# kotaro-kinoshita/yomitoku

Measured on AMD Instinct MI355X. Metric: pages/sec (DocumentAnalyzer @1600x1200, lite model set), higher is better.
Workload: dtype f32 held as two scaled fp16 planes per operand on the MFMA pipe: 3 x v_mfma_f32_32x32x16_f16 per product tile (products to 2^-21, below the fp32 accumulation's own rounding), fp32 accumulate, fp32 activations in HBM; attention, LayerNorm, the fused greedy step and every grid-starved launch exact fp3

## Files before the change

yomitoku_amd/csrc/ymk_api.cpp:

```cpp
#include "../../include/ymk.h"
#include "ymk_common.h"
#include "ymk_decstep.h"
#include "ymk_det.h"
#include "ymk_entry.h"
#include "ymk_seq.h"

struct ymk_model {
  ymk::Model* impl = nullptr;
  int device = 0;
};

#include <dlfcn.h>
namespace {
struct Roctx {
  int (*push)(const char*) = nullptr;
  int (*pop)() = nullptr;
  Roctx() {
    const char* on = std::getenv("YMK_ROCTX");
    if (on == nullptr || on[0] == '\0' || on[0] == '0') return;
    for (const char* name : {"librocprofiler-sdk-roctx.so", "libroctx64.so"}) {
      if (void* h = dlopen(name, RTLD_NOW | RTLD_GLOBAL)) {
        push = reinterpret_cast<int (*)(const char*)>(dlsym(h, "roctxRangePushA"));
        pop = reinterpret_cast<int (*)()>(dlsym(h, "roctxRangePop"));
        if (push && pop) return;
// ... 26 lines not shown
    return 1;                                       \
  }                                                 \
  catch (...) {                                     \
    ymk::set_error("unknown C++ exception");        \
    return 2;                                       \
  }

extern "C" {

int ymk_version(void) { return 100; }

const char* ymk_last_error(void) { return ymk::last_error().c_str(); }

int ymk_device_count(void) {
  int n = 0;
  if (hipGetDeviceCount(&n) != hipSuccess) return -1;
  return n;
}

ymk_model* ymk_model_create(const char* kind, int device) {
  try {
    YMK_CHECK(kind != nullptr, "kind is null");
    YMK_HIP(hipSetDevice(device));
    std::string k(kind);
    ymk::Model* impl = nullptr;
    if (k == "dbnet") impl = ymk::create_dbnet();
    else if (k == "parseq") impl = ymk::create_parseq();
    else if (k == "rtdetr") impl = ymk::create_rtdetr();
    else throw ymk::Error("unknown model kind: " + k);
    auto* m = new ymk_model();
    m->impl = impl;
    m->device = device;
    return m;
  } catch (const std::exception& e) {
    ymk::set_error(e.what());
    return nullptr;
  }
}

void ymk_model_destroy(ymk_model* m) {
  if (!m) return;
  (void)hipSetDevice(m->device);
  delete m->impl;
  delete m;
}

int ymk_model_set_param(ymk_model* m, const char* key, double value) {
  YMK_API_BEGIN
  YMK_CHECK(m && key, "null argument");
  const std::string k(key);
  if (k == "workspace_reuse") {
    YMK_CHECK(value == 0.0 || value == 1.0 || value == -1.0, "workspace_reuse must be 0 or 1 (-1: follow the process-wide default)");
    YMK_CHECK(!ymk::in_forward(), "workspace_reuse cannot change inside a forward");
  }
  m->impl->params[key] = value;
  if (m->impl->finalized && (k == "conv_split" || k == "conv_split_encoder")) {
    YMK_HIP(hipSetDevice(m->device));
    m->impl->prebuild_split();
  }
  YMK_API_END
}

int ymk_model_set_tensor(ymk_model* m, const char* name, const float* host_data, int ndim, const int64_t* dims) {
  YMK_API_BEGIN
  YMK_CHECK(m && name && host_data && (ndim == 0 || dims), "null argument");
  YMK_CHECK(!m->impl->finalized, "model already finalized");
  m->impl->ws.put(name, host_data, ndim, dims);
  YMK_API_END
}

int ymk_model_finalize(ymk_model* m) {
  YMK_API_BEGIN
  RoctxRange roctx_range("ymk_model_finalize");
  YMK_CHECK(m, "null model");
  YMK_HIP(hipSetDevice(m->device));
  m->impl->finalize();
  m->impl->prebuild_split();
  if (!ymk::debug_hazard_no_finalize_sync()) YMK_HIP(hipDeviceSynchronize());
  YMK_API_END
}

int ymk_model_reserve(ymk_model* m, int n, int h, int w, void* stream) {
  YMK_API_BEGIN
  RoctxRange roctx_range("ymk_model_reserve");
  YMK_CHECK(m && m->impl, "null argument");
  YMK_HIP(hipSetDevice(m->device));
  m->impl->reserve(n, h, w, (hipStream_t)stream);
  YMK_API_END
}

int64_t ymk_model_weight_bytes(const ymk_model* m) { return m ? (int64_t)m->impl->pool.bytes() : -1; }
int64_t ymk_model_workspace_bytes(const ymk_model* m) { return m ? (int64_t)m->impl->arena.capacity() : -1; }

int ymk_dbnet_forward(ymk_model* m, const float* x_dev, int n, int h, int w, float* prob_dev, void* stream) {
  YMK_API_BEGIN
  RoctxRange roctx_range("ymk_dbnet_forward");
  YMK_CHECK(m && x_dev && prob_dev, "null argument");
  YMK_HIP(hipSetDevice(m->device));
  ymk::dbnet_forward(m->impl, x_dev, n, h, w, prob_dev, (hipStream_t)stream);
  YMK_API_END
}

int ymk_parseq_dims(ymk_model* m, int* num_steps, int* num_classes) {
  YMK_API_BEGIN
  YMK_CHECK(m && num_steps && num_classes, "null argument");
  ymk::parseq_dims(m->impl, num_steps, num_classes);
  YMK_API_END
}

int ymk_parseq_forward(ymk_model* m, const float* x_dev, int b, int w, float* logits_dev, int* out_len, int* ar_steps,
                       void* stream) {
  YMK_API_BEGIN
  RoctxRange roctx_range("ymk_parseq_forward");
  YMK_CHECK(m && x_dev && logits_dev && out_len && ar_steps, "null argument");
  YMK_HIP(hipSetDevice(m->device));
  ymk::parseq_forward(m->impl, x_dev, b, w, logits_dev, out_len, ar_steps, (hipStream_t)stream);
  YMK_API_END
}

int ymk_parseq_forward_groups(ymk_model* m, const float* const* x_dev, const int* b, const int* w, int n_groups,
                              float* logits_dev, int* out_len, int* ar_steps, void* stream) {
  YMK_API_BEGIN
  RoctxRange roctx_range("ymk_parseq_forward_groups");
  YMK_CHECK(m && x_dev && b && w && logits_dev && out_len && ar_steps, "null argument");
  YMK_HIP(hipSetDevice(m->device));
  ymk::parseq_forward_groups(m->impl, x_dev, b, w, n_groups, logits_dev, out_len, ar_steps, (hipStream_t)stream);
  YMK_API_END
}

int ymk_parseq_token_stats(const float* logits_dev, int rows, int num_classes, int* ids_dev, float* probs_dev,
                           void* stream) {
  YMK_API_BEGIN
  RoctxRange roctx_range("ymk_parseq_token_stats");
  YMK_CHECK(logits_dev && ids_dev && probs_dev, "null argument");
  ymk::row_maxprob((hipStream_t)stream, logits_dev, rows, num_classes, ids_dev, probs_dev);
  YMK_API_END
}

int ymk_rtdetr_forward(ymk_model* m, const float* x_dev, int b, int h, int w, float* logits_dev, float* boxes_dev,
                       void* stream) {
  YMK_API_BEGIN
  RoctxRange roctx_range("ymk_rtdetr_forward");
  YMK_CHECK(m && x_dev && logits_dev && boxes_dev, "null argument");
  YMK_HIP(hipSetDevice(m->device));
  ymk::rtdetr_forward(m->impl, x_dev, b, h, w, logits_dev, boxes_dev, (hipStream_t)stream);
  YMK_API_END
}

int ymk_debug_option(const char* key, int value) {
  YMK_API_BEGIN
  YMK_CHECK(key != nullptr, "null key");
  const std::string k(key);
  YMK_CHECK(ymk::conv_debug_option(k, value) || ymk::parseq_debug_option(k, value) || ymk::decstep_debug_option(k, value) ||
                ymk::conv_split_debug_option(k, value) || ymk::runtime_debug_option(k, value),
            "unknown debug option: " + k);
  YMK_API_END
}

int ymk_stat(const char* key, int64_t* value) {
  YMK_API_BEGIN
  YMK_CHECK(key != nullptr && value != nullptr, "null argument");
  long long v = 0;
  YMK_CHECK(ymk::conv_split_stat(std::string(key), &v) || ymk::runtime_stat(std::string(key), &v) || ymk::parseq_stat(std::string(key), &v), std::string("unknown counter: ") + key);
  *value = v;
  YMK_API_END
}

int ymk_amax_check_counters(int64_t* out4) {
  YMK_API_BEGIN
  YMK_CHECK(out4 != nullptr, "null argument");
  long long v[4];
  ymk::amax_check_counters(v);
  for (int i = 0; i < 4; ++i) out4[i] = v[i];
  YMK_API_END
}

int ymk_prof_begin(void) {
  YMK_API_BEGIN
  ymk::prof_begin();
  YMK_API_END
}

int ymk_prof_end(double* conv_ms, double* conv_flop, int64_t* conv_launches) {
  YMK_API_BEGIN
  YMK_CHECK(conv_ms && conv_flop && conv_launches, "null argument");
  ymk::prof_end(conv_ms, conv_flop, conv_launches);
  YMK_API_END
}

int ymk_prof_bytes(double* conv_bytes) {
  YMK_API_BEGIN
  YMK_CHECK(conv_bytes, "null argument");
  *conv_bytes = ymk::prof_bytes();
  YMK_API_END
}

int ymk_prof_launch_table(double* ms, double* flop, double* bytes, double* mfma_products, int64_t capacity, int64_t* count) {
  YMK_API_BEGIN
  YMK_CHECK(count != nullptr && capacity >= 0 && (capacity == 0 || (ms && flop && bytes && mfma_products)), "null argument");
  *count = ymk::prof_launch_table(ms, flop, bytes, mfma_products, capacity);
  YMK_API_END
}

int ymk_op_plan_workspace(int64_t n, const int64_t* sizes, const int64_t* release_pos, int64_t* offsets_out, int64_t* peak_out,
                          int64_t* live_bound_out) {
  YMK_API_BEGIN
  YMK_CHECK(n >= 0 && (n == 0 || (sizes && offsets_out)), "plan_workspace: bad argument");
  std::vector<size_t> sz((size_t)n), off((size_t)n);
  for (int64_t k = 0; k < n; ++k) {
    YMK_CHECK(sizes[k] >= 0, "plan_workspace: negative size");
    sz[(size_t)k] = (size_t)sizes[k];
  }
  size_t peak = 0, live = 0;
  ymk::plan_workspace((size_t)n, sz.data(), release_pos, off.data(), &peak, &live);
  for (int64_t k = 0; k < n; ++k) offsets_out[k] = (int64_t)off[(size_t)k];
  if (peak_out) *peak_out = (int64_t)peak;
  if (live_bound_out) *live_bound_out = (int64_t)live;
  YMK_API_END
}

int ymk_op_conv2d(const float* x_dev, int n, int h, int w, int c, const float* w_host_oihw, int cout, int cin, int kh,
                  int kw, const float* scale_host, const float* bias_host, const float* res_dev, int stride, int pad,
                  int dil, int act, int tap4, float* y_dev, void* stream) {
  YMK_API_BEGIN
  using namespace ymk;
  DevicePool pool;
  ConvW cw;
  cw.cout = cout;
  cw.cin = tap4 ? 4 : cin;
  cw.kh = kh;
  cw.kw = kw;
  cw.mode = tap4 ? 1 : 0;
  std::vector<float> panel;
  pack_conv_weight(w_host_oihw, cout, cin, kh, kw, tap4 != 0, panel, cw.kpad, cw.ctiles);
  cw.w = pool.upload(panel);
  if (scale_host) cw.scale = pool.upload(scale_host, cout);
  if (bias_host) cw.bias = pool.upload(bias_host, cout);
  Tensor in{const_cast<float*>(x_dev), n, h, w, c, c};
  const int oh = conv_out_dim(h, kh, stride, pad, dil), ow = conv_out_dim(w, kw, stride, pad, dil);
  Tensor out{y_dev, n, oh, ow, cout, cout};
  Tensor res{const_cast<float*>(res_dev), n, oh, ow, cout, cout};
  ConvArgs a;
  a.stride = stride;
  a.pad = pad;
  a.dil = dil;
  a.act = act;
  a.res = res_dev ? &res : nullptr;
  SplitCtxOwner split_ctx;
  ConvSplitScope scope(-1, split_ctx.get(), 0);
  conv2d((hipStream_t)stream, in, cw, a, out);
  YMK_HIP(hipStreamSynchronize((hipStream_t)stream));
  YMK_API_END
}

static ymk::ConvW op_conv_weight(ymk::DevicePool& pool, const float* w_host_oihw, int cout, int cin, int kh, int kw, bool tap4,
                                 const float* scale_host, const float* bias_host) {
  using namespace ymk;
  ConvW cw;
  cw.cout = cout;
  cw.cin = tap4 ? 4 : cin;
  cw.kh = kh;
  cw.kw = kw;
  cw.mode = tap4 ? 1 : 0;
  std::vector<float> panel;
  pack_conv_weight(w_host_oihw, cout, cin, kh, kw, tap4, panel, cw.kpad, cw.ctiles);
  cw.w = pool.upload(panel);
  std::vector<float> scale, bias;
  if (scale_host) scale.assign(scale_host, scale_host + cout);
  if (bias_host) bias.assign(bias_host, bias_host + cout);
  if (scale_host) cw.scale = pool.upload(scale);
  if (bias_host) cw.bias = pool.upload(bias);
  plane_bound(cw, w_host_oihw, (size_t)cin * kh * kw, scale, bias);
  return cw;
}

int ymk_op_conv2d_view(const float* x_dev, int n, int h, int w, int c, int in_ld, const float* w_host_oihw, int cout, int kh, int kw,
                       int tap4, const float* scale_host, const float* bias_host, const float* res_dev, int res_ld, int res_post,
                       int stride_h, int stride_w, int pad, int dil, int act, const int* row_group_dev, const int* group_open_dev,
                       const unsigned* amax_in_dev, unsigned* amax_out_dev, float* y_dev, int out_ld, void* stream) {
  YMK_API_BEGIN
  using namespace ymk;
  YMK_CHECK(x_dev && w_host_oihw && y_dev, "null argument");
  YMK_CHECK(n > 0 && h > 0 && w > 0 && c > 0 && in_ld > 0 && cout > 0 && kh > 0 && kw > 0 && res_ld >= 0 && out_ld > 0 &&
                stride_h > 0 && stride_w > 0 && pad >= 0 && dil > 0,
            "conv2d_view: sizes, strides and leading dimensions are positive (res_ld may be 0)");
  hipStream_t s = (hipStream_t)stream;
  DevicePool pool;
  const ConvW cw = op_conv_weight(pool, w_host_oihw, cout, c, kh, kw, tap4 != 0, scale_host, bias_host);
  SplitCtxOwner split_ctx;
  ConvSplitScope scope(-1, split_ctx.get(), 0);
  if (row_group_dev || group_open_dev) {
    YMK_CHECK(kh == 1 && kw == 1 && stride_h == 1 && stride_w == 1 && pad == 0 && !res_post && !tap4,
              "conv2d_view: a row predicate comes with a plain linear layer");
    gemm(s, x_dev, n * h * w, c, in_ld, cw, act, res_dev, res_ld, y_dev, out_ld, row_group_dev, group_open_dev, EPI_STORE, amax_in_dev,
         amax_out_dev);
  } else {
    Tensor in{const_cast<float*>(x_dev), n, h, w, c, in_ld};
    const int oh = conv_out_dim(h, kh, stride_h, pad, dil), ow = conv_out_dim(w, kw, stride_w, pad, dil);
    Tensor out{y_dev, n, oh, ow, cout, out_ld};
    Tensor res{const_cast<float*>(res_dev), n, oh, ow, cout, res_ld};
    ConvArgs a;
    a.stride = stride_h;
    a.stride_w = stride_w;
    a.pad = pad;
    a.dil = dil;
    a.act = act;
    a.res = res_dev ? &res : nullptr;
    a.res_post = res_post != 0;
    a.amax_in = amax_in_dev;
    a.amax_out = amax_out_dev;
    conv2d(s, in, cw, a, out);
  }
  YMK_HIP(hipStreamSynchronize(s));
  YMK_API_END
}

// ... 515 lines not shown
```

yomitoku_amd/csrc/ymk_seq.h:

```cpp
#pragma once
#include "ymk_common.h"

namespace ymk {

void layernorm(hipStream_t s, const float* x, int ldx, int in_rows_mod, const float* g, const float* b, float eps,
               float* y, int ldy, int M, int D);
void add_pos_embed(hipStream_t s, float* x, const float* pos, int B, int gh, int gw, int full_gw, int D);

struct SeqTab {
  const int *qoff = nullptr, *qlen = nullptr, *koff = nullptr, *klen = nullptr;
};

void flash_attention(hipStream_t s, const float* q, const float* k, const float* v, float* o, int B, int H, int Lq, int Lk,
                     int hd, int ldq, int ldk, int ldv, int ldo, long bsq, long bsk, long bsv, long bso, float scale,
                     const SeqTab* tab = nullptr, const unsigned* amax_q = nullptr, const unsigned* amax_k = nullptr,
                     const unsigned* amax_v = nullptr);
void small_attention(hipStream_t s, const float* q, const float* k, const float* v, float* o, int B, int H, int Lq, int Lk,
                     int hd, int ldq, int ldk, int ldv, int ldo, long bsq, long bsk, long bsv, long bso, float scale,
                     const unsigned char* mask_qk, int ld_mask, const unsigned char* kpm, int ld_kpm,
                     const SeqTab* tab = nullptr);
void nar_cross_attention(hipStream_t s, const float* q, const float* k, const float* v, float* o, int B, int H, int Lq, int Lk,
                         int hd, int ldq, int ldk, int ldv, int ldo, long bsk, long bsv, long bso, float scale,
                         const SeqTab* tab = nullptr);
void init_decode(hipStream_t s, int* tok, int ld_tok, int* state, int bos_id, int pad_id, int B);

void ctx_embed_ln(hipStream_t s, const int* tok, int ld_tok, int pos0, int npos, const float* emb, const float* posq,
                  const float* g, const float* be, float eps, float* out, int out_rows, int D, int B);
void greedy_step(hipStream_t s, const float* logits, long ld_b, int C, int step, int num_steps, int* tok, int* raw,
                 int ld_tok, int* state, int eos_id, int rep_on, int period_max, int min_run_p1, int min_repeats,
                 int* not_done, const int* prev_not_done, int* arrived, int* host_flag, int B, const int* gid = nullptr,
                 int* gopen = nullptr, int ng = 1, int partials = 0);
void publish_open(hipStream_t s, const int* not_done, const int* prev_not_done, int* host_flag);
void refine_prep(hipStream_t s, const int* raw, int ld_tok, int S, int bos_id, int eos_id, int* tok2, unsigned char* kpm,
                 int B, const int* gid = nullptr, const int* gsteps = nullptr);
void row_argmax(hipStream_t s, const float* logits, int rows, int C, int* out);
void rep_cut(hipStream_t s, float* logits, long ld_b, int C, int S, const int* state, int eos_id, int B);
void row_maxprob(hipStream_t s, const float* logits, int rows, int C, int* ids, float* probs);
void tile_rows(hipStream_t s, const float* src, int rows, int D, float* dst, int B);
void fill_i32(hipStream_t s, int* p, int v, size_t n);

}
```

yomitoku_amd/csrc/ymk_seq.hip:

```cpp
#include "ymk_common.h"
#include "ymk_f16_planes.h"
#include "ymk_seq.h"

namespace ymk {


__device__ __forceinline__ float wave_sum(float v) {
#pragma unroll
  for (int o = 32; o > 0; o >>= 1) v += __shfl_xor(v, o, 64);
  return v;
}
__device__ __forceinline__ float wave_max(float v) {
#pragma unroll
  for (int o = 32; o > 0; o >>= 1) v = fmaxf(v, __shfl_xor(v, o, 64));
  return v;
}

__global__ void k_layernorm(const float* __restrict__ x, int ldx, int in_rows_mod, const float* __restrict__ g,
                            const float* __restrict__ b, float eps, float* __restrict__ y, int ldy, int M, int D) {
  const int row = blockIdx.x * (blockDim.x >> 6) + (threadIdx.x >> 6);
  const int lane = threadIdx.x & 63;
  if (row >= M) return;
  const float* xr = x + (size_t)(in_rows_mod > 0 ? row % in_rows_mod : row) * ldx;
  float4 v[4];
  const int nv = D >> 2;
  float s = 0.f;
#pragma unroll
  for (int i = 0; i < 4; ++i) {
    const int c = lane + 64 * i;
    if (c < nv) {
      v[i] = *reinterpret_cast<const float4*>(xr + c * 4);
      s += (v[i].x + v[i].y) + (v[i].z + v[i].w);
    }
  }
  const float mean = wave_sum(s) / (float)D;
  float q = 0.f;
#pragma unroll
  for (int i = 0; i < 4; ++i) {
    const int c = lane + 64 * i;
    if (c < nv) {
      const float a = v[i].x - mean, bb = v[i].y - mean, cc = v[i].z - mean, d = v[i].w - mean;
      q += (a * a + bb * bb) + (cc * cc + d * d);
    }
  }
  const float rstd = 1.f / sqrtf(wave_sum(q) / (float)D + eps);
#pragma unroll
  for (int i = 0; i < 4; ++i) {
    const int c = lane + 64 * i;
    if (c < nv) {
      const float4 gg = *reinterpret_cast<const float4*>(g + c * 4);
      const float4 be = *reinterpret_cast<const float4*>(b + c * 4);
      float4 o;
      o.x = (v[i].x - mean) * rstd * gg.x + be.x;
      o.y = (v[i].y - mean) * rstd * gg.y + be.y;
      o.z = (v[i].z - mean) * rstd * gg.z + be.z;
      o.w = (v[i].w - mean) * rstd * gg.w + be.w;
      *reinterpret_cast<float4*>(y + (size_t)row * ldy + c * 4) = o;
    }
  }
}
void layernorm(hipStream_t s, const float* x, int ldx, int in_rows_mod, const float* g, const float* b, float eps,
               float* y, int ldy, int M, int D) {
  YMK_CHECK(D % 4 == 0 && D <= 1024, "layernorm: D must be a multiple of 4, <= 1024");
  if (M == 0) return;
  hipLaunchKernelGGL(k_layernorm, dim3((M + 3) / 4), dim3(256), 0, s, x, ldx, in_rows_mod, g, b, eps, y, ldy, M, D);
  YMK_HIP(hipGetLastError());
}

__global__ void k_add_pos(float* __restrict__ x, const float* __restrict__ pos, int gh, int gw, int full_gw, int D4,
                          size_t total) {
  for (size_t i = (size_t)blockIdx.x * blockDim.x + threadIdx.x; i < total; i += (size_t)gridDim.x * blockDim.x) {
    const int c4 = (int)(i % D4);
    const size_t tok = i / D4;
    const int cc = (int)(tok % gw);
    const int rr = (int)((tok / gw) % gh);
    float4 v = reinterpret_cast<float4*>(x)[i];
    const float4 p = reinterpret_cast<const float4*>(pos)[(size_t)(rr * full_gw + cc) * D4 + c4];
    v.x += p.x; v.y += p.y; v.z += p.z; v.w += p.w;
    reinterpret_cast<float4*>(x)[i] = v;
  }
}
void add_pos_embed(hipStream_t s, float* x, const float* pos, int B, int gh, int gw, int full_gw, int D) {
  const size_t total = (size_t)B * gh * gw * (D / 4);
  size_t g = (total + 255) / 256;
  if (g > 4096) g = 4096;
  hipLaunchKernelGGL(k_add_pos, dim3((int)g), dim3(256), 0, s, x, pos, gh, gw, full_gw, D / 4, total);
  YMK_HIP(hipGetLastError());
}

struct AttnP {
  const float *q, *k, *v;
  float* o;
  int ldq, ldk, ldv, ldo;
  long bsq, bsk, bsv, bso;
  int Lq, Lk, H;
  float scale;
  const int *qoff, *qlen, *koff, *klen;
  const unsigned *amax_q, *amax_k, *amax_v;
};

template <int HD, int HDR = HD>
__global__ __launch_bounds__(256, 1) void k_flash_attn(AttnP p) {
  constexpr int KT = 64;
  constexpr int LDH = HD + 4;
  constexpr int NKC = HDR / 8;
  constexpr int NDC = HD / 32;
  constexpr int LPT = (KT * HDR / 4) / 256;
  static_assert(HD % 32 == 0 && HDR % 8 == 0 && HDR <= HD && (KT * HDR / 4) % 256 == 0, "head dim");
  __shared__ __attribute__((aligned(16))) float lds[2 * 2 * KT * LDH];

  const int t = threadIdx.x, wv = t >> 6, lane = t & 63, li = lane & 31, lh = lane >> 5;
  const int b = blockIdx.z, h = blockIdx.y;
  const int q0 = blockIdx.x * 128 + wv * 32;
  const float* qb = p.q + (size_t)b * p.bsq + h * HDR;
  const float* kb = p.k + (size_t)b * p.bsk + h * HDR;
  const float* vb = p.v + (size_t)b * p.bsv + h * HDR;
  float* ob = p.o + (size_t)b * p.bso + h * HDR;
  int Lq = p.Lq, Lk = p.Lk;
  if (p.koff) {
    const size_t r = (size_t)p.koff[b];
    kb = p.k + r * p.ldk + h * HDR;
    vb = p.v + r * p.ldv + h * HDR;
    Lk = p.klen[b];
  }
  if (p.qoff) {
    const size_t r = (size_t)p.qoff[b];
    qb = p.q + r * p.ldq + h * HDR;
    ob = p.o + r * p.ldo + h * HDR;
    Lq = p.qlen[b];
  }
  if ((int)blockIdx.x * 128 >= Lq) return;

  f32x4 qf[NKC];
  {
    const int qi = min(q0 + li, Lq - 1);
    const float* qr = qb + (size_t)qi * p.ldq;
#pragma unroll
    for (int kc = 0; kc < NKC; ++kc) {
      qf[kc] = *reinterpret_cast<const f32x4*>(qr + kc * 8 + lh * 4);
      qf[kc] *= p.scale;
    }
  }

  f32x16 oacc[NDC];
#pragma unroll
  for (int dc = 0; dc < NDC; ++dc)
#pragma unroll
    for (int r = 0; r < 16; ++r) oacc[dc][r] = 0.f;
  float m_run = -INFINITY, l_run = 0.f;

  f32x4 rk[LPT], rv[LPT];
  auto load_kv = [&](int k0) {
// ... 172 lines not shown
    for (int i = 0; i < LPT; ++i) {
      const int idx = t + 256 * i;
      const int row = idx / (HDR / 4), c4 = idx - row * (HDR / 4);
      *reinterpret_cast<f32x4*>(Ks + row * LDH + c4 * 4) = rk[i];
      *reinterpret_cast<f32x4*>(Vs + row * LDH + c4 * 4) = rv[i];
    }
  };

  const int ntiles = (Lk + KT - 1) / KT;
  load_kv(0);
  store_kv(0);
  __syncthreads();
  for (int tt = 0; tt < ntiles; ++tt) {
    const int buf = tt & 1;
    if (tt + 1 < ntiles) load_kv((tt + 1) * KT);
    const float* Ks = lds + buf * (2 * KT * LDH);
    const float* Vs = Ks + KT * LDH;
#pragma unroll
    for (int sub = 0; sub < (q0 < Lq ? KT / 32 : 0); ++sub) {
      const int kbase = tt * KT + sub * 32;
      if (kbase >= Lk) break;
      f32x16 sacc;
#pragma unroll
      for (int r = 0; r < 16; ++r) sacc[r] = 0.f;
      const float* kr = Ks + (sub * 32 + li) * LDH + lh * 8;
#pragma unroll
      for (int ks = 0; ks < NKS; ++ks) {
        const f32x4 a = *reinterpret_cast<const f32x4*>(kr + ks * 16);
        const f32x4 c = *reinterpret_cast<const f32x4*>(kr + ks * 16 + 4);
        const float x[8] = {a.x, a.y, a.z, a.w, c.x, c.y, c.z, c.w};
        f16x8 kh, kl;
        f16_split8(x, s_k, kh, kl);
        sacc = __builtin_amdgcn_mfma_f32_32x32x16_f16(kl, qh[ks], sacc, 0, 0, 0);
        sacc = __builtin_amdgcn_mfma_f32_32x32x16_f16(kh, ql[ks], sacc, 0, 0, 0);
        sacc = __builtin_amdgcn_mfma_f32_32x32x16_f16(kh, qh[ks], sacc, 0, 0, 0);
      }
      float mt = -INFINITY;
#pragma unroll
      for (int r = 0; r < 16; ++r) {
        const int key = kbase + (r & 3) + 8 * (r >> 2) + 4 * lh;
        sacc[r] = key >= Lk ? -INFINITY : sacc[r] * s_unscale;
        mt = fmaxf(mt, sacc[r]);
      }
      mt = fmaxf(mt, __shfl_xor(mt, 32, 64));
      const float m_new = fmaxf(m_run, mt);
      const float alpha = __expf(m_run - m_new);
      float ps = 0.f;
#pragma unroll
      for (int r = 0; r < 16; ++r) {
        sacc[r] = __expf(sacc[r] - m_new);
        ps += sacc[r];
      }
      ps += __shfl_xor(ps, 32, 64);
      l_run = l_run * alpha + ps;
      m_run = m_new;
      f16x8 ph[2], pl[2];
#pragma unroll
      for (int j = 0; j < 2; ++j) {
        const float x[8] = {sacc[8 * j], sacc[8 * j + 1], sacc[8 * j + 2], sacc[8 * j + 3], sacc[8 * j + 4], sacc[8 * j + 5], sacc[8 * j + 6], sacc[8 * j + 7]};
        f16_split8(x, 16384.f, ph[j], pl[j]);
      }
#pragma unroll
      for (int dc = 0; dc < NDC; ++dc) {
#pragma unroll
        for (int r = 0; r < 16; ++r) oacc[dc][r] *= alpha;
        const float* vr = Vs + (sub * 32 + 4 * lh) * LDH + dc * 32 + li;
#pragma unroll
        for (int j = 0; j < 2; ++j) {
          float x[8];
#pragma unroll
          for (int e = 0; e < 8; ++e) {
            const int r = 8 * j + e;
            x[e] = vr[((r & 3) + 8 * (r >> 2)) * LDH];
          }
          f16x8 vh, vl;
          f16_split8(x, s_v, vh, vl);
          oacc[dc] = __builtin_amdgcn_mfma_f32_32x32x16_f16(vl, ph[j], oacc[dc], 0, 0, 0);
          oacc[dc] = __builtin_amdgcn_mfma_f32_32x32x16_f16(vh, pl[j], oacc[dc], 0, 0, 0);
          oacc[dc] = __builtin_amdgcn_mfma_f32_32x32x16_f16(vh, ph[j], oacc[dc], 0, 0, 0);
        }
      }
    }
    if (tt + 1 < ntiles) store_kv(buf ^ 1);
    __syncthreads();
  }
  const int qi = q0 + li;
  if (qi < Lq) {
    const float inv = o_unscale / l_run;
    float* orow = ob + (size_t)qi * p.ldo;
#pragma unroll
    for (int dc = 0; dc < NDC; ++dc)
#pragma unroll
      for (int g = 0; g < 4; ++g) {
        f32x4 w;
        w.x = oacc[dc][4 * g + 0] * inv;
        w.y = oacc[dc][4 * g + 1] * inv;
        w.z = oacc[dc][4 * g + 2] * inv;
        w.w = oacc[dc][4 * g + 3] * inv;
        if (dc * 32 + 8 * g + 4 * lh < HDR) *reinterpret_cast<f32x4*>(orow + dc * 32 + 8 * g + 4 * lh) = w;
      }
  }
}

void flash_attention(hipStream_t s, const float* q, const float* k, const float* v, float* o, int B, int H, int Lq, int Lk,
                     int hd, int ldq, int ldk, int ldv, int ldo, long bsq, long bsk, long bsv, long bso, float scale,
                     const SeqTab* tab, const unsigned* amax_q, const unsigned* amax_k, const unsigned* amax_v) {
  if (B == 0 || Lq == 0) return;
  YMK_CHECK(Lk > 0, "attention: no keys");
  YMK_CHECK(ldq % 4 == 0 && ldk % 4 == 0 && ldv % 4 == 0 && ldo % 4 == 0, "attention: strides must be multiples of 4");
  AttnP p{q, k, v, o, ldq, ldk, ldv, ldo, bsq, bsk, bsv, bso, Lq, Lk, H, scale, nullptr, nullptr, nullptr, nullptr, amax_q, amax_k, amax_v};
  if (tab) {
    p.qoff = tab->qoff;
    p.qlen = tab->qlen;
    p.koff = tab->koff;
    p.klen = tab->klen;
    YMK_CHECK((p.qoff == nullptr) == (p.qlen == nullptr) && (p.koff == nullptr) == (p.klen == nullptr), "attention: offset and length tables come in pairs");
  }
  dim3 grid((Lq + 127) / 128, H, B);
  const bool f16 = amax_q && amax_k && amax_v && scale <= 1.f && scale > 0.f && conv_effective_split() == SPLIT_F16X2 && ldq % 4 == 0;
  if (f16 && (hd == 32 || hd == 64 || hd == 96 || hd == 48)) {
    if (hd == 32) hipLaunchKernelGGL(k_flash_attn_f16<32>, grid, dim3(256), 0, s, p);
    else if (hd == 64) hipLaunchKernelGGL(k_flash_attn_f16<64>, grid, dim3(256), 0, s, p);
    else if (hd == 96) hipLaunchKernelGGL(k_flash_attn_f16<96>, grid, dim3(256), 0, s, p);
    else hipLaunchKernelGGL((k_flash_attn_f16<64, 48>), grid, dim3(256), 0, s, p);
    YMK_HIP(hipGetLastError());
    return;
  }
  if (hd == 32) hipLaunchKernelGGL(k_flash_attn<32>, grid, dim3(256), 0, s, p);
  else if (hd == 64) hipLaunchKernelGGL(k_flash_attn<64>, grid, dim3(256), 0, s, p);
  else if (hd == 96) hipLaunchKernelGGL(k_flash_attn<96>, grid, dim3(256), 0, s, p);
  else if (hd == 48) hipLaunchKernelGGL((k_flash_attn<64, 48>), grid, dim3(256), 0, s, p);
  else {
    YMK_CHECK(Lk <= 1024 && hd <= 128, "attention: head dim " + std::to_string(hd) + " is only supported for <= 1024 keys per sample");
    small_attention(s, q, k, v, o, B, H, Lq, Lk, hd, ldq, ldk, ldv, ldo, bsq, bsk, bsv, bso, scale, nullptr, 0, nullptr, 0, tab);
    return;
  }
  YMK_HIP(hipGetLastError());
}

struct SmallAttnP {
  const float *q, *k, *v;
  float* o;
  int ldq, ldk, ldv, ldo;
  long bsq, bsk, bsv, bso;
  int Lq, Lk, H, hd;
  float scale;
  const unsigned char* mask_qk;
  int ld_mask;
  const unsigned char* kpm;
  int ld_kpm;
  const int *koff, *klen;
  const int *qoff, *qlen;
  int vec4;
};
__global__ __launch_bounds__(64) void k_small_attn(SmallAttnP p) {
  __shared__ float prob[1024];
  __shared__ float qs[128];
  const int lane = threadIdx.x;
  const int qi = blockIdx.x, h = blockIdx.y, b = blockIdx.z;
  if (p.qoff && qi >= p.qlen[b]) return;
  const size_t qrow0 = p.qoff ? (size_t)p.qoff[b] : 0;
  const float* qr = (p.qoff ? p.q + qrow0 * p.ldq : p.q + (size_t)b * p.bsq) + (size_t)qi * p.ldq + h * p.hd;
  for (int d = lane; d < p.hd; d += 64) qs[d] = qr[d] * p.scale;
  __syncthreads();
  const float* kb = p.k + (size_t)b * p.bsk + h * p.hd;
  const float* vb = p.v + (size_t)b * p.bsv + h * p.hd;
  int Lk = p.Lk;
  if (p.koff) {
    kb = p.k + (size_t)p.koff[b] * p.ldk + h * p.hd;
    vb = p.v + (size_t)p.koff[b] * p.ldv + h * p.hd;
    Lk = p.klen[b];
  }
  float mx = -INFINITY;
  for (int k = lane; k < Lk; k += 64) {
    bool blocked = false;
    if (p.mask_qk) blocked = p.mask_qk[(size_t)qi * p.ld_mask + k] != 0;
    if (p.kpm) blocked = blocked || p.kpm[(size_t)b * p.ld_kpm + k] != 0;
    float sc = -INFINITY;
    if (!blocked) {
      const float* kr = kb + (size_t)k * p.ldk;
      float a = 0.f;
      if (p.vec4) {
        for (int d = 0; d < p.hd; d += 4) {
          const float4 kk = *reinterpret_cast<const float4*>(kr + d);
          a += qs[d] * kk.x + qs[d + 1] * kk.y + qs[d + 2] * kk.z + qs[d + 3] * kk.w;
        }
      } else {
        for (int d = 0; d < p.hd; ++d) a += qs[d] * kr[d];
      }
      sc = a;
    }
    prob[k] = sc;
    mx = fmaxf(mx, sc);
  }
  mx = wave_max(mx);
  float sum = 0.f;
  for (int k = lane; k < Lk; k += 64) {
    const float e = __expf(prob[k] - mx);
    prob[k] = e;
    sum += e;
  }
  sum = wave_sum(sum);
  __syncthreads();
  const float inv = 1.f / sum;
  float* orow = (p.qoff ? p.o + qrow0 * p.ldo : p.o + (size_t)b * p.bso) + (size_t)qi * p.ldo + h * p.hd;
  for (int d = lane; d < p.hd; d += 64) {
    float a = 0.f;
    for (int k = 0; k < Lk; ++k) a += prob[k] * vb[(size_t)k * p.ldv + d];
    orow[d] = a * inv;
  }
}
void small_attention(hipStream_t s, const float* q, const float* k, const float* v, float* o, int B, int H, int Lq, int Lk,
                     int hd, int ldq, int ldk, int ldv, int ldo, long bsq, long bsk, long bsv, long bso, float scale,
                     const unsigned char* mask_qk, int ld_mask, const unsigned char* kpm, int ld_kpm, const SeqTab* tab) {
  if (B == 0 || Lq == 0) return;
  YMK_CHECK(Lk > 0 && Lk <= 1024 && hd <= 128, "small attention: Lk <= 1024, hd <= 128");
  const int vec4 = hd % 4 == 0 && ldk % 4 == 0 && bsk % 4 == 0 && ((uintptr_t)k & 15) == 0;
  SmallAttnP p{q, k, v, o, ldq, ldk, ldv, ldo, bsq, bsk, bsv, bso, Lq, Lk, H, hd, scale, mask_qk, ld_mask, kpm, ld_kpm,
               tab ? tab->koff : nullptr, tab ? tab->klen : nullptr, tab ? tab->qoff : nullptr, tab ? tab->qlen : nullptr, vec4};
  YMK_CHECK(!tab || (!mask_qk && !kpm), "small attention: ragged batches come without masks");
  hipLaunchKernelGGL(k_small_attn, dim3(Lq, H, B), dim3(64), 0, s, p);
  YMK_HIP(hipGetLastError());
}

__global__ void k_ctx_embed_ln(const int* __restrict__ tok, int ld_tok, int pos0, int npos, const float* __restrict__ emb,
                               const float* __restrict__ posq, const float* __restrict__ g, const float* __restrict__ be,
                               float eps, float sqrt_d, float* __restrict__ out, int out_rows, int D, int B) {
  const int w = blockIdx.x * (blockDim.x >> 6) + (threadIdx.x >> 6);
  const int lane = threadIdx.x & 63;
  if (w >= B * npos) return;
  const int b = w / npos, pos = pos0 + (w - b * npos);
  const int token = tok[(size_t)b * ld_tok + pos];
  const float* er = emb + (size_t)token * D;
  const float* pr = pos > 0 ? posq + (size_t)(pos - 1) * D : nullptr;
  float v[16];
  float s = 0.f;
  const int per = (D + 63) / 64;
  for (int i = 0; i < per; ++i) {
    const int c = lane + 64 * i;
    float x = 0.f;
    if (c < D) {
      x = sqrt_d * er[c];
      if (pr) x = pr[c] + x;
      s += x;
    }
    v[i] = x;
  }
  const float mean = wave_sum(s) / (float)D;
  float q = 0.f;
  for (int i = 0; i < per; ++i) {
    const int c = lane + 64 * i;
    if (c < D) q += (v[i] - mean) * (v[i] - mean);
  }
  const float rstd = 1.f / sqrtf(wave_sum(q) / (float)D + eps);
  float* orow = out + ((size_t)b * out_rows + pos) * D;
  for (int i = 0; i < per; ++i) {
    const int c = lane + 64 * i;
    if (c < D) orow[c] = (v[i] - mean) * rstd * g[c] + be[c];
  }
}
void ctx_embed_ln(hipStream_t s, const int* tok, int ld_tok, int pos0, int npos, const float* emb, const float* posq,
                  const float* g, const float* be, float eps, float* out, int out_rows, int D, int B) {
  YMK_CHECK(D <= 1024, "ctx_embed: D <= 1024");
  const int waves = B * npos;
  if (waves == 0) return;
  hipLaunchKernelGGL(k_ctx_embed_ln, dim3((waves + 3) / 4), dim3(256), 0, s, tok, ld_tok, pos0, npos, emb, posq, g, be, eps,
                     sqrtf((float)D), out, out_rows, D, B);
  YMK_HIP(hipGetLastError());
}

constexpr int ROW_RV = 32;
template <bool WITH_SUM>
__device__ __forceinline__ void row_reduce_256(const float* __restrict__ row, int C, float* sv, int* si, float& mx, int& am,
                                               float& sum) {
  const int t = threadIdx.x;
  float best = -INFINITY;
  int bi = t < C ? t : 0x7fffffff;
  float v[ROW_RV];
  const bool in_regs = C <= 256 * ROW_RV;
  if (in_regs) {
#pragma unroll
    for (int i = 0; i < ROW_RV; ++i) {
      const int c = t + 256 * i;
      v[i] = c < C ? row[c] : -INFINITY;
    }
#pragma unroll
    for (int i = 0; i < ROW_RV; ++i)
      if (v[i] > best) {
        best = v[i];
        bi = t + 256 * i;
      }
  } else {
    for (int c = t; c < C; c += 256) {
      const float x = row[c];
      if (x > best) {
        best = x;
        bi = c;
      }
    }
  }
  sv[t] = best;
  si[t] = bi;
  __syncthreads();
  for (int o = 128; o > 0; o >>= 1) {
    if (t < o) {
      const float v2 = sv[t + o];
      const int i2 = si[t + o];
      if (v2 > sv[t] || (v2 == sv[t] && i2 < si[t])) {
        sv[t] = v2;
        si[t] = i2;
      }
    }
    __syncthreads();
  }
  mx = sv[0];
  am = si[0];
  if (WITH_SUM) {
    __syncthreads();
    float acc = 0.f;
    if (in_regs) {
#pragma unroll
      for (int i = 0; i < ROW_RV; ++i)
        if (t + 256 * i < C) acc += expf(v[i] - mx);
    } else {
      for (int c = t; c < C; c += 256) acc += expf(row[c] - mx);
    }
    sv[t] = acc;
    __syncthreads();
    for (int o = 128; o > 0; o >>= 1) {
      if (t < o) sv[t] += sv[t + o];
      __syncthreads();
    }
    sum = sv[0];
  }
}

__global__ __launch_bounds__(256) void k_greedy_step(const float* __restrict__ logits, long ld_b, int C, int step,
                                                     int num_steps, int* __restrict__ tok, int* __restrict__ raw,
                                                     int ld_tok, int* __restrict__ state, int eos_id, int rep_on,
                                                     int period_max, int min_run_p1, int min_repeats,
                                                     int* __restrict__ not_done, const int* __restrict__ prev_not_done,
                                                     int* __restrict__ arrived, int* __restrict__ host_flag,
                                                     const int* __restrict__ gid, int* __restrict__ gopen, int ng, int partials,
                                                     int flags) {
  const int b = blockIdx.x, t = threadIdx.x;
  if (prev_not_done && *prev_not_done == 0) return;
  const int g = gid ? gid[b] : 0;
  const bool frozen = gid && step > 0 && gopen[(size_t)(step - 1) * ng + g] == 0;
  __shared__ float sv[256];
  __shared__ int si[256];
  if (!frozen && !partials) {
    float mx, unused;
    int am;
    row_reduce_256<false>(logits + (size_t)b * ld_b, C, sv, si, mx, am, unused);
  }
  if (!frozen && partials) {
    const float2* pr = reinterpret_cast<const float2*>(logits + (size_t)b * ld_b);
    float v = -INFINITY;
    int i = 0x7fffffff;
    if (t < C) {
      const float2 q = pr[t];
      v = q.x;
      i = __float_as_int(q.y);
    }
    sv[t] = v;
    si[t] = i;
    __syncthreads();
    for (int o = 128; o > 0; o >>= 1) {
      if (t < o) {
        const float v2 = sv[t + o];
        const int i2 = si[t + o];
        if (v2 > sv[t] || (v2 == sv[t] && i2 < si[t])) {
          sv[t] = v2;
// ... 200 lines not shown
```

Baseline: 129.4.

## Stage K/V in LDS and process multiple queries per wave in small attention

Adds a staged small-attention kernel that launches one block per (head, batch), copies the whole K and V slice into LDS once, and has each wave handle several query rows. It reuses the LDS-resident K/V across all queries and shares each V load across 2–4 queries in the PV loop. The goal is to avoid re-reading K/V from global memory for every query, which the old one-block-per-query kernel did. The cost is much less grid parallelism (H*B blocks instead of Lq*H*B) and LDS use up to 64KB that can limit occupancy. A debug option falls back to the old path.

```diff
diff --git a/yomitoku_amd/csrc/ymk_api.cpp b/yomitoku_amd/csrc/ymk_api.cpp
--- a/yomitoku_amd/csrc/ymk_api.cpp
+++ b/yomitoku_amd/csrc/ymk_api.cpp
@@ -202,7 +202,7 @@
   YMK_CHECK(key != nullptr, "null key");
   const std::string k(key);
   YMK_CHECK(ymk::conv_debug_option(k, value) || ymk::parseq_debug_option(k, value) || ymk::decstep_debug_option(k, value) ||
-                ymk::conv_split_debug_option(k, value) || ymk::runtime_debug_option(k, value),
+                ymk::conv_split_debug_option(k, value) || ymk::runtime_debug_option(k, value) || ymk::seq_debug_option(k, value),
             "unknown debug option: " + k);
   YMK_API_END
 }
@@ -211,7 +211,8 @@
   YMK_API_BEGIN
   YMK_CHECK(key != nullptr && value != nullptr, "null argument");
   long long v = 0;
-  YMK_CHECK(ymk::conv_split_stat(std::string(key), &v) || ymk::runtime_stat(std::string(key), &v) || ymk::parseq_stat(std::string(key), &v), std::string("unknown counter: ") + key);
+  YMK_CHECK(ymk::conv_split_stat(std::string(key), &v) || ymk::runtime_stat(std::string(key), &v) || ymk::parseq_stat(std::string(key), &v) || ymk::seq_stat(std::string(key), &v),
+            std::string("unknown counter: ") + key);
   *value = v;
   YMK_API_END
 }
diff --git a/yomitoku_amd/csrc/ymk_seq.h b/yomitoku_amd/csrc/ymk_seq.h
--- a/yomitoku_amd/csrc/ymk_seq.h
+++ b/yomitoku_amd/csrc/ymk_seq.h
@@ -19,6 +19,8 @@
                      int hd, int ldq, int ldk, int ldv, int ldo, long bsq, long bsk, long bsv, long bso, float scale,
                      const unsigned char* mask_qk, int ld_mask, const unsigned char* kpm, int ld_kpm,
                      const SeqTab* tab = nullptr);
+bool seq_debug_option(const std::string& key, int value);
+bool seq_stat(const std::string& key, long long* value);
 void nar_cross_attention(hipStream_t s, const float* q, const float* k, const float* v, float* o, int B, int H, int Lq, int Lk,
                          int hd, int ldq, int ldk, int ldv, int ldo, long bsk, long bsv, long bso, float scale,
                          const SeqTab* tab = nullptr);
diff --git a/yomitoku_amd/csrc/ymk_seq.hip b/yomitoku_amd/csrc/ymk_seq.hip
--- a/yomitoku_amd/csrc/ymk_seq.hip
+++ b/yomitoku_amd/csrc/ymk_seq.hip
@@ -1,3 +1,5 @@
+#include <atomic>
+
 #include "ymk_common.h"
 #include "ymk_f16_planes.h"
 #include "ymk_seq.h"
@@ -476,16 +478,88 @@
   const int *koff, *klen;
   const int *qoff, *qlen;
   int vec4;
+  int vec4v;
 };
+__device__ __forceinline__ void small_attn_load_q(float* qs, const float* qr, int hd, float scale, int lane) {
+  for (int d = lane; d < hd; d += 64) qs[d] = qr[d] * scale;
+}
+__device__ __forceinline__ float small_attn_softmax(const SmallAttnP& p, int qi, int b, int lane, const float* qs, float* prob,
+                                                    const float* kb, int ldk, int Lk) {
+  qs = static_cast<const float*>(__builtin_assume_aligned(qs, 16));
+  float mx = -INFINITY;
+  for (int k = lane; k < Lk; k += 64) {
+    unsigned char mq = 0, mk = 0;
+    if (p.mask_qk) mq = p.mask_qk[(size_t)qi * p.ld_mask + k];
+    if (p.kpm) mk = p.kpm[(size_t)b * p.ld_kpm + k];
+    const bool blocked = (mq | mk) != 0;
+    float sc = -INFINITY;
+    if (!blocked) {
+      const float* kr = kb + (size_t)k * ldk;
+      float a = 0.f;
+      if (p.vec4) {
+        kr = static_cast<const float*>(__builtin_assume_aligned(kr, 16));
+#pragma unroll 4
+        for (int d = 0; d < p.hd; d += 4) {
+          const float4 kk = *reinterpret_cast<const float4*>(kr + d);
+          a += qs[d] * kk.x + qs[d + 1] * kk.y + qs[d + 2] * kk.z + qs[d + 3] * kk.w;
+        }
+      } else {
+        for (int d = 0; d < p.hd; ++d) a += qs[d] * kr[d];
+      }
+      sc = a;
+    }
+    prob[k] = sc;
+    mx = fmaxf(mx, sc);
+  }
+  mx = wave_max(mx);
+  float sum = 0.f;
+  for (int k = lane; k < Lk; k += 64) {
+    const float e = __expf(prob[k] - mx);
+    prob[k] = e;
+    sum += e;
+  }
+  return wave_sum(sum);
+}
+template <int NQ>
+__device__ __forceinline__ void small_attn_pv(const float* prob, int ldp, const float* vb, int ldv, int Lk, int hd, int d0, int dstep,
+                                              const float (&inv)[NQ], float* const (&orow)[NQ]) {
+  for (int d = d0; d < hd; d += dstep) {
+    float a[NQ];
+#pragma unroll
+    for (int j = 0; j < NQ; ++j) a[j] = 0.f;
+    int k = 0;
+#pragma unroll 2
+    for (; k + 4 <= Lk; k += 4) {
+      const float v0 = vb[(size_t)k * ldv + d], v1 = vb[(size_t)(k + 1) * ldv + d];
+      const float v2 = vb[(size_t)(k + 2) * ldv + d], v3 = vb[(size_t)(k + 3) * ldv + d];
+#pragma unroll
+      for (int j = 0; j < NQ; ++j) {
+        const float4 pj = *static_cast<const float4*>(__builtin_assume_aligned(prob + j * ldp + k, 16));
+        a[j] = fmaf(pj.x, v0, a[j]);
+        a[j] = fmaf(pj.y, v1, a[j]);
+        a[j] = fmaf(pj.z, v2, a[j]);
+        a[j] = fmaf(pj.w, v3, a[j]);
+      }
+    }
+    for (; k < Lk; ++k) {
+      const float v = vb[(size_t)k * ldv + d];
+#pragma unroll
+      for (int j = 0; j < NQ; ++j) a[j] = fmaf(prob[j * ldp + k], v, a[j]);
+    }
+#pragma unroll
+    for (int j = 0; j < NQ; ++j)
+      if (orow[j]) orow[j][d] = a[j] * inv[j];
+  }
+}
 __global__ __launch_bounds__(64) void k_small_attn(SmallAttnP p) {
-  __shared__ float prob[1024];
-  __shared__ float qs[128];
+  __shared__ __attribute__((aligned(16))) float prob[1024];
+  __shared__ __attribute__((aligned(16))) float qs[128];
   const int lane = threadIdx.x;
   const int qi = blockIdx.x, h = blockIdx.y, b = blockIdx.z;
   if (p.qoff && qi >= p.qlen[b]) return;
   const size_t qrow0 = p.qoff ? (size_t)p.qoff[b] : 0;
   const float* qr = (p.qoff ? p.q + qrow0 * p.ldq : p.q + (size_t)b * p.bsq) + (size_t)qi * p.ldq + h * p.hd;
-  for (int d = lane; d < p.hd; d += 64) qs[d] = qr[d] * p.scale;
+  small_attn_load_q(qs, qr, p.hd, p.scale, lane);
   __syncthreads();
   const float* kb = p.k + (size_t)b * p.bsk + h * p.hd;
   const float* vb = p.v + (size_t)b * p.bsv + h * p.hd;
@@ -495,54 +569,126 @@
     vb = p.v + (size_t)p.koff[b] * p.ldv + h * p.hd;
     Lk = p.klen[b];
   }
-  float mx = -INFINITY;
-  for (int k = lane; k < Lk; k += 64) {
-    bool blocked = false;
-    if (p.mask_qk) blocked = p.mask_qk[(size_t)qi * p.ld_mask + k] != 0;
-    if (p.kpm) blocked = blocked || p.kpm[(size_t)b * p.ld_kpm + k] != 0;
-    float sc = -INFINITY;
-    if (!blocked) {
-      const float* kr = kb + (size_t)k * p.ldk;
-      float a = 0.f;
-      if (p.vec4) {
-        for (int d = 0; d < p.hd; d += 4) {
-          const float4 kk = *reinterpret_cast<const float4*>(kr + d);
-          a += qs[d] * kk.x + qs[d + 1] * kk.y + qs[d + 2] * kk.z + qs[d + 3] * kk.w;
-        }
-      } else {
-        for (int d = 0; d < p.hd; ++d) a += qs[d] * kr[d];
-      }
-      sc = a;
-    }
-    prob[k] = sc;
-    mx = fmaxf(mx, sc);
-  }
-  mx = wave_max(mx);
-  float sum = 0.f;
-  for (int k = lane; k < Lk; k += 64) {
-    const float e = __expf(prob[k] - mx);
-    prob[k] = e;
-    sum += e;
-  }
-  sum = wave_sum(sum);
+  const float sum = small_attn_softmax(p, qi, b, lane, qs, prob, kb, p.ldk, Lk);
   __syncthreads();
-  const float inv = 1.f / sum;
-  float* orow = (p.qoff ? p.o + qrow0 * p.ldo : p.o + (size_t)b * p.bso) + (size_t)qi * p.ldo + h * p.hd;
-  for (int d = lane; d < p.hd; d += 64) {
-    float a = 0.f;
-    for (int k = 0; k < Lk; ++k) a += prob[k] * vb[(size_t)k * p.ldv + d];
-    orow[d] = a * inv;
-  }
-}
+  const float inv[1] = {1.f / sum};
+  float* const orow[1] = {(p.qoff ? p.o + qrow0 * p.ldo : p.o + (size_t)b * p.bso) + (size_t)qi * p.ldo + h * p.hd};
+  small_attn_pv<1>(prob, 0, vb, p.ldv, Lk, p.hd, lane, 64, inv, orow);
+}
+
+__device__ __forceinline__ void wave_lds_fence() {
+  __builtin_amdgcn_fence(__ATOMIC_RELEASE, "wavefront");
+  __builtin_amdgcn_wave_barrier();
+  __builtin_amdgcn_fence(__ATOMIC_ACQUIRE, "wavefront");
+}
+constexpr int SMALL_ATTN_QPL = 2;
+template <int HALVES>
+__global__ __launch_bounds__(512) void k_small_attn_staged(SmallAttnP p, int ldl, int lkp, int hdp) {
+  constexpr int QPL = SMALL_ATTN_QPL, QPW = HALVES * QPL;
+  extern __shared__ float4 small_attn_lds4[];
+  const int tid = threadIdx.x, nthr = blockDim.x, lane = tid & 63, wave = tid >> 6, nw = nthr >> 6;
+  const int h = blockIdx.x, b = blockIdx.y;
+  const int Lk = p.Lk, hd = p.hd;
+  float* Ks = reinterpret_cast<float*>(small_attn_lds4);
+  float* Vs = Ks + Lk * ldl;
+  float* prob = Vs + Lk * ldl + wave * (QPW * lkp + hdp);
+  float* qs = prob + QPW * lkp;
+  const float* kb = p.k + (size_t)b * p.bsk + h * hd;
+  const float* vb = p.v + (size_t)b * p.bsv + h * hd;
+  if (p.vec4) {
+    const int n4 = hd >> 2;
+    for (int i = tid; i < Lk * n4; i += nthr) {
+      const int r = i / n4, c = (i - r * n4) * 4;
+      *reinterpret_cast<float4*>(Ks + r * ldl + c) = *reinterpret_cast<const float4*>(kb + (size_t)r * p.ldk + c);
+    }
+  } else {
+    for (int i = tid; i < Lk * hd; i += nthr) {
+      const int r = i / hd, c = i - r * hd;
+      Ks[r * ldl + c] = kb[(size_t)r * p.ldk + c];
+    }
+  }
+  if (p.vec4v) {
+    const int n4 = hd >> 2;
+    for (int i = tid; i < Lk * n4; i += nthr) {
+      const int r = i / n4, c = (i - r * n4) * 4;
+      *reinterpret_cast<float4*>(Vs + r * ldl + c) = *reinterpret_cast<const float4*>(vb + (size_t)r * p.ldv + c);
+    }
+  } else {
+    for (int i = tid; i < Lk * hd; i += nthr) {
+      const int r = i / hd, c = i - r * hd;
+      Vs[r * ldl + c] = vb[(size_t)r * p.ldv + c];
+    }
+  }
+  __syncthreads();
+  const float* qb = p.q + (size_t)b * p.bsq + h * hd;
+  float* ob = p.o + (size_t)b * p.bso + h * hd;
+  for (int q0 = wave * QPW; q0 < p.Lq; q0 += nw * QPW) {
+    float inv[QPW];
+#pragma unroll
+    for (int j = 0; j < QPW; ++j) {
+      inv[j] = 0.f;
+      const int qi = q0 + j;
+      if (qi < p.Lq) {
+        small_attn_load_q(qs, qb + (size_t)qi * p.ldq, hd, p.scale, lane);
+        wave_lds_fence();
+        inv[j] = 1.f / small_attn_softmax(p, qi, b, lane, qs, prob + j * lkp, Ks, ldl, Lk);
+        wave_lds_fence();
+      }
+    }
+    const int g = HALVES == 2 ? lane >> 5 : 0;
+    float invl[QPL];
+    float* orow[QPL];
+#pragma unroll
+    for (int i = 0; i < QPL; ++i) {
+      const int qi = q0 + g * QPL + i;
+      invl[i] = inv[i];
+      if constexpr (HALVES == 2) {
+        if (g) invl[i] = inv[QPL + i];
+      }
+      orow[i] = qi < p.Lq ? ob + (size_t)qi * p.ldo : nullptr;
+    }
+    small_attn_pv<QPL>(prob + g * QPL * lkp, lkp, Vs, ldl, Lk, hd, HALVES == 2 ? lane & 31 : lane, 64 / HALVES, invl, orow);
+    wave_lds_fence();
+  }
+}
+
+static std::atomic<int> g_small_attn_staged{1};
+static std::atomic<long long> g_small_attn_staged_launches{0};
+bool seq_debug_option(const std::string& key, int value) {
+  if (key != "small_attn_staged") return false;
+  g_small_attn_staged = value;
+  return true;
+}
+bool seq_stat(const std::string& key, long long* value) {
+  if (key != "small_attn_staged_launches") return false;
+  *value = g_small_attn_staged_launches.load();
+  return true;
+}
+constexpr size_t SMALL_ATTN_LDS_MAX = 64 * 1024;
 void small_attention(hipStream_t s, const float* q, const float* k, const float* v, float* o, int B, int H, int Lq, int Lk,
                      int hd, int ldq, int ldk, int ldv, int ldo, long bsq, long bsk, long bsv, long bso, float scale,
                      const unsigned char* mask_qk, int ld_mask, const unsigned char* kpm, int ld_kpm, const SeqTab* tab) {
   if (B == 0 || Lq == 0) return;
   YMK_CHECK(Lk > 0 && Lk <= 1024 && hd <= 128, "small attention: Lk <= 1024, hd <= 128");
   const int vec4 = hd % 4 == 0 && ldk % 4 == 0 && bsk % 4 == 0 && ((uintptr_t)k & 15) == 0;
+  const int vec4v = hd % 4 == 0 && ldv % 4 == 0 && bsv % 4 == 0 && ((uintptr_t)v & 15) == 0;
   SmallAttnP p{q, k, v, o, ldq, ldk, ldv, ldo, bsq, bsk, bsv, bso, Lq, Lk, H, hd, scale, mask_qk, ld_mask, kpm, ld_kpm,
-               tab ? tab->koff : nullptr, tab ? tab->klen : nullptr, tab ? tab->qoff : nullptr, tab ? tab->qlen : nullptr, vec4};
+               tab ? tab->koff : nullptr, tab ? tab->klen : nullptr, tab ? tab->qoff : nullptr, tab ? tab->qlen : nullptr, vec4, vec4v};
   YMK_CHECK(!tab || (!mask_qk && !kpm), "small attention: ragged batches come without masks");
+  if (Lq >= 2 && !tab && (size_t)Lk * hd * 2 * sizeof(float) <= SMALL_ATTN_LDS_MAX && B <= 65535 &&
+      g_small_attn_staged.load(std::memory_order_relaxed) != 0) {
+    const int hdp = (hd + 3) & ~3, lkp = (Lk + 3) & ~3, ldl = hdp + 4;
+    const int qpw = (hd <= 32 ? 2 : 1) * SMALL_ATTN_QPL;
+    const int nw = (size_t)2 * Lk * ldl * sizeof(float) > 32 * 1024 ? 8 : 4;
+    const size_t lds = ((size_t)2 * Lk * ldl + (size_t)nw * (qpw * lkp + hdp)) * sizeof(float);
+    if (lds <= SMALL_ATTN_LDS_MAX) {
+      if (hd <= 32) hipLaunchKernelGGL(k_small_attn_staged<2>, dim3(H, B), dim3(64 * nw), lds, s, p, ldl, lkp, hdp);
+      else hipLaunchKernelGGL(k_small_attn_staged<1>, dim3(H, B), dim3(64 * nw), lds, s, p, ldl, lkp, hdp);
+      YMK_HIP(hipGetLastError());
+      ++g_small_attn_staged_launches;
+      return;
+    }
+  }
   hipLaunchKernelGGL(k_small_attn, dim3(Lq, H, B), dim3(64), 0, s, p);
   YMK_HIP(hipGetLastError());
 }
```

Result: slower. 124.8 (-3.6%).
